# lukasc-ch/CBinfer

Hardware: AMD Instinct MI355X
Metric: frames/sec + effective GFLOP/s vs dense, scene-labeling CNN 480x320 @10% change (higher is better)
Workload: dtype f32-equivalent: f32 tensors, every operand as three bf16 terms (24 bits, exact), six products on the bf16 MFMA, f32 accumulate; 1 GPU; sceneLabeling CBConv2d coarse-grained fp32, synthetic 480x320 seq @10% change (32x32 re-drawn blocks), experiment 6, one sequence per GPU; sequences_per_gpu=1, launch=program

## Files before the change

cbinfer_amd/csrc/cb_split.hip:

```cpp
#include <stdlib.h>

#include <type_traits>

#include "cb_common.h"

#ifdef CBS_STAMP
__device__ unsigned long long cbs_stamp_buf[4 * 2048 * 16];
#define CB_TAIL_STAMP(i)                                                                 \
    do {                                                                                 \
        if (threadIdx.x == 0 && blockIdx.x < 2048)                                       \
            cbs_stamp_buf[(2 * 2048 + blockIdx.x) * 16 + (i)] = __builtin_amdgcn_s_memrealtime(); \
    } while (0)
#define CBS_DET_STAMP(i)                                                                                            \
    do {                                                                                                            \
        const unsigned wg = blockIdx.y * gridDim.x + blockIdx.x;                                                    \
        if (POOL && threadIdx.x == 0 && blockIdx.z == 0 && wg < 2048)                                               \
            cbs_stamp_buf[(3 * 2048 + wg) * 16 + (i)] = __builtin_amdgcn_s_memrealtime();                            \
    } while (0)
#else
#define CBS_DET_STAMP(i)
#endif
#include "cb_tail_core.h"
#include "cb_split_common.h"

namespace cbs {

typedef __attribute__((address_space(3))) void* cb_lds_ptr;

__global__ __launch_bounds__(256) void cbs_prep_kernel(const float* __restrict__ w, halfx8* __restrict__ A,
                                                      int* __restrict__ stageOff, float* __restrict__ wPlain,
                                                      CbsGeom g, int K, int KP, float wscale) {
    const long idx = (long)blockIdx.x * blockDim.x + threadIdx.x;
    if (wPlain)
        for (long i = idx; i < (long)K * g.C * g.kH * g.kW; i += (long)gridDim.x * blockDim.x) wPlain[i] = w[i];
    const int PL = g.planes;
    if (idx < g.nStages) {
        const int s = (int)idx;
        int off;
        if (g.pair) {
            off = ((s / g.kWs) * g.Wp + 2 * (s % g.kWs)) * g.rec;
// ... 240 lines not shown
struct CbsSeq {
    const char* S;
    const float* state;
    const int* rangeFlag;
    float* out;
    unsigned long long* masks;
    int32_t* listOut;
    int32_t* countOut;
    unsigned long long* maskCopy;
    float* reluOut;
};
struct CbsParams {
    CbsSeq seq[CBS_MAXSEQ];
    int nSeq;
    const char* A;
    const int* stageOff;
    const float* wPlain;
    const float* bias;
    float* slabs;
    int* info;
    int slabCap;
    int K, KP, H, W, Wp, rec, nStages, maskWords, wpr, relu, dummyBase, kH, kW;
    long stateBytes, aBytes;
    float outScale;
    unsigned long long magicMW, magicWpr, magicW, magicMT;
    int arriveShards;
    int forceSK;
    int accumulate;
    int splitRounds;
    int halfOut;
    const int* upstream;
    int dbg;
    int maxChunks;
};
static __device__ __forceinline__ const void* cbs_uniform_ptr(const void* ptr) {
    const unsigned long a = (unsigned long)ptr;
    const unsigned lo = (unsigned)__builtin_amdgcn_readfirstlane((int)(unsigned)a);
    const unsigned hi = (unsigned)__builtin_amdgcn_readfirstlane((int)(unsigned)(a >> 32));
    return (const void*)(((unsigned long)hi << 32) | lo);
}
#define CBH_GROUP CBINFER_HGROUP_MAX
#define CBH_NEXT CBINFER_HNEXT_MAX
struct CbhNext {
    _Float16* state;
    char* S;
    unsigned long long* masks;
    int kHH, kWH, Wp, rec, padY, padXL;
    float th;
    int pad_;
};
struct CbhLayer {
    const char* A;
    const _Float16* bias;
    int K, relu, nNext, pad_;
    CbhNext next[CBH_NEXT];
};
struct CbhExt {
    CbhLayer L[CBH_GROUP];
    int slabCap1;
    int pad_;
};
struct CbsNoExt {};
struct CbsWinExt {
    float* nstate;
    char* nS;
    unsigned long long* nmasks;
// ... 18 lines not shown
struct CbsExtOf<3> {
    typedef CbsWinExt type;
};
struct CbsSideExt {
    const float* sideFrame;
    float* sideState;
    int sideC, sideHW;
    float sideTh;
};
template <>
struct CbsExtOf<4> {
    typedef CbsSideExt type;
};

__device__ __forceinline__ void cbh_or_dilated(unsigned long long* masks, int y, int x, int H, int W, int wpr, int kHH,
                                               int kWH) {
    const int lo = max(x - kWH, 0), hi = min(x + kWH, W - 1);
    const int w0 = lo >> 6, w1 = hi >> 6;
    const unsigned long long m0 = (~0ull << (lo & 63)) & (w1 == w0 ? (~0ull >> (63 - (hi & 63))) : ~0ull);
    const unsigned long long m1 = ~0ull >> (63 - (hi & 63));
    for (int yy = max(y - kHH, 0); yy <= min(y + kHH, H - 1); ++yy) {
        atomicOr(&masks[(long)yy * wpr + w0], m0);
        if (w1 != w0) atomicOr(&masks[(long)yy * wpr + w1], m1);
    }
}

#ifdef CBS_STAMP
#define CBS_STAMP_AT(i)                                                                                   \
    do {                                                                                                  \
        if (threadIdx.x == 0 && blockIdx.x < 2048 && cbs_first)                                           \
            cbs_stamp_buf[(BM >= 128 ? 2048 * 16 : 0) + blockIdx.x * 16 + (i)] =                            \
                ((i) == 6 || (i) == 7) ? __builtin_amdgcn_s_memtime() : __builtin_amdgcn_s_memrealtime();               \
    } while (0)
#else
#define CBS_STAMP_AT(i)
#endif
#ifdef CBS_DBG
#define CBS_DBGBIT(b) (p.dbg & (b))
#else
#define CBS_DBGBIT(b) false
#endif
#define CBS_INFO_SK 0
#define CBS_INFO_MT 1
#define CBS_INFO_TP 4
#define CBS_INFO_CH 24

template <int OFF>
__device__ __forceinline__ void cbs_dma16(__amdgpu_buffer_rsrc_t rsrc, char* lds, int voff, int soff) {
    __builtin_amdgcn_raw_ptr_buffer_load_lds(rsrc, (cb_lds_ptr)lds, 16, voff, soff, OFF, 0);
}

template <int OFF>
__device__ __forceinline__ halfx8 cbs_lds_read16(unsigned addr) {
    halfx8 v;
    asm volatile("ds_read_b128 %0, %1 offset:%2" : "=v"(v) : "v"(addr), "n"(OFF));
    return v;
}

__device__ __forceinline__ int cbs_div(int x, unsigned long long magic) {
    return (int)(((unsigned long long)(unsigned)x * magic) >> 32);
}

template <int BM, int BN, int WM, int WN, int PRE_CAP, bool MASK_LDS, int RING, int AR = 0>
__global__ __launch_bounds__(64 * WM * WN) void cbs_conv_kernel(CbsParams p, typename CbsExtOf<AR>::type ext) {
    constexpr bool HALF = AR == 1, X3 = AR == 2 || AR == 3 || AR == 4, WIN = AR == 3, SIDE = AR == 3 || AR == 4;
    if (HALF && p.upstream && *p.upstream == 0) {
        if (blockIdx.x == 0 && threadIdx.x == 0) {
            p.seq[0].countOut[0] = 0;
            if (p.info) p.info[CBS_INFO_SK] = 1;
        }
        return;
    }
    cb_touch_kernarg<sizeof(CbsParams) + (HALF ? sizeof(CbhExt) : (WIN ? sizeof(CbsWinExt) : (SIDE ? sizeof(CbsSideExt) : 0)))>();
    constexpr int NW = WM * WN, NT = 64 * NW;
    constexpr int TN = BN / WN / 32;
    static_assert(BM == 32 * WM, "one 32-row tile per wave");
    constexpr int PB = X3 ? 192 : 128;
    constexpr int ABLK = BM * PB / 1024, BBLK = BN * PB / 1024;
    constexpr int APW = ABLK / NW, BPW = BBLK / NW;
    static_assert(APW * NW == ABLK && BPW * NW == BBLK && APW >= 1 && BPW >= 1, "DMA blocks must deal evenly");
    constexpr int DPW = APW + BPW;
    constexpr int A_BYTES = BM * PB, B_BYTES = BN * PB, STAGE = A_BYTES + B_BYTES;
    constexpr int TILE = BM * BN;
    __shared__ __attribute__((aligned(1024))) char ring[RING * STAGE];
    __shared__ int s_pre[PRE_CAP + 1];
    __shared__ unsigned long long s_mask[MASK_LDS ? PRE_CAP : 1];
    __shared__ const unsigned long long* s_maskPtr[CBS_MAXSEQ];
    __shared__ int s_wsum[NW];
    __shared__ int s_tilePix[BN];
    __shared__ float s_bias[BM];
    __shared__ unsigned s_nchg[HALF ? CBH_NEXT * (BN / 32) : 1];
    __shared__ int s_preW[WIN ? PRE_CAP / 2 + 2 : 1];
    __shared__ int s_tileAny[WIN ? BN : 1];
    __shared__ int s_winPos[WIN ? BN / 4 : 1];
    __shared__ unsigned s_wchg;
    __shared__ unsigned long long s_wsum64[WIN ? 64 * WM * WN / 64 : 1];
    static_assert(!WIN || (BN / WN / 32 == 1 && MASK_LDS), "window order: one column tile per wave, the mask words in LDS");

    const int t = threadIdx.x;
    const int lane = t & 63, wave = __builtin_amdgcn_readfirstlane(t >> 6);
    const int wm = wave % WM, wn = wave / WM;
    const int l31 = lane & 31, h = lane >> 5;
// ... 401 lines not shown
                    v += outx[(long)m * HWx + pix];
                    float* rp = pp->seq[q].reluOut;
                    if (rp) rp[(long)m * HWx + pix] = v <= 0.f ? 0.f : v;
                }
                outx[(long)m * HWx + pix] = v;
            }
            continue;
        }

        const char* Sq = p.seq[q].S;
        const int bRecords = (int)min(p.stateBytes + CBS_SPAD, (long)0x7fffffff);
        const int aVoff = wave * APW * 1024 + lane * 16;
        int bVoff[BPW];
#pragma unroll
        for (int i = 0; i < BPW; ++i) {
            const int nl = X3 ? wave * 16 + (lane >> 2) : (wave * BPW + i) * 8 + (lane >> 3);
            const int pos = s_tilePix[nl];
            const int py = cbs_div(max(pos, 0), p.magicW);
            const int base = (pos < 0 || CBS_DBGBIT(1)) ? p.dummyBase : (py * p.Wp + (pos - py * p.W)) * p.rec;
            if (X3)
                bVoff[i] = CBS_SPAD + base + ((i * 4 + ((lane & 3) ^ ((lane >> 4) & 3))) << 4) - i * 1024;
            else
                bVoff[i] = CBS_SPAD + base + (((lane & 7) ^ ((nl >> 1) & 7)) << 4) - (APW + i) * 1024;
        }
        const int aItem = (m0 / 32) * (PB * 32);
        const int aStageBytes = (p.KP / 32) * (PB * 32);

        CBS_STAMP_AT(11);
        __amdgpu_buffer_rsrc_t isA, isB;
        char* isMine = ring;
        int isAS = 0, isBS = 0;
        auto issue = [&](int s, bool setUpOnly = false) {
            char* dst = ring + (s % RING) * STAGE;
            const bool live = s < sEnd;
            const int aS = live ? s * aStageBytes + aItem : 0;
            const int bS = bNext;
            bNext = stageOff[min(s + 1, sEnd - 1)];
            if (CBS_DBGBIT(4)) return;
            const __amdgpu_buffer_rsrc_t ar = __builtin_amdgcn_make_buffer_rsrc(
                (void*)Aq, 0, (live && !CBS_DBGBIT(64 | 128)) ? aRecords : 0, 0x00020000);
            const __amdgpu_buffer_rsrc_t br = __builtin_amdgcn_make_buffer_rsrc(
                (void*)Sq, 0, (live && !CBS_DBGBIT(64 | 256)) ? bRecords : 0, 0x00020000);
            char* mine = dst + wave * (DPW * 1024);
            if (setUpOnly) {
                isA = ar, isB = br, isMine = mine, isAS = aS, isBS = bS;
                return;
            }
            if constexpr (X3) {
                cbs_dma16<0>(ar, mine, aVoff, aS);
                cbs_dma16<1024>(ar, mine, aVoff, aS);
                cbs_dma16<2048>(ar, mine, aVoff, aS);
                cbs_dma16<0>(br, mine + 3072, bVoff[0], bS);
                cbs_dma16<1024>(br, mine + 3072, bVoff[BPW > 1 ? 1 : 0], bS);
                cbs_dma16<2048>(br, mine + 3072, bVoff[BPW > 2 ? 2 : 0], bS);
            } else {
                cbs_dma16<0>(ar, mine, aVoff, aS);
                cbs_dma16<1024>(ar, mine, aVoff, aS);
                cbs_dma16<2048>(br, mine, bVoff[0], bS);
                cbs_dma16<3072>(br, mine, bVoff[1], bS);
            }
        };

        auto issuePart = [&](auto partTag) {
            constexpr int I = decltype(partTag)::value;
            if (CBS_DBGBIT(4)) return;
            if constexpr (X3) {
                if constexpr (I == 0) cbs_dma16<0>(isA, isMine, aVoff, isAS);
// ... 186 lines not shown
                asm volatile("s_waitcnt lgkmcnt(0)"
                             : "+v"(f.a[0]), "+v"(f.a[1]), "+v"(f.a[2]), "+v"(f.a[3]), "+v"(f.b[0]), "+v"(f.b[1]),
                               "+v"(f.b[2]), "+v"(f.b[3])
                             :
                             : "memory");
        };
#define CBS_SB() __builtin_amdgcn_sched_barrier(0)
#define CBS_STEP(WAITN, ISSUE, S, FCUR, FNEXT)                                            \
        do {                                                                               \
            asm volatile("s_waitcnt vmcnt(%0)" ::"n"(WAITN) : "memory");                  \
            __builtin_amdgcn_s_barrier();                                                  \
            CBS_SB();                                                                      \
            if (ISSUE) issue((S) + RING, true);                                            \
            CBS_SB();                                                                      \
            mmaRange(FCUR, 0, 1); CBS_SB(); if (ISSUE) issuePart(P0()); CBS_SB();          \
            mmaRange(FCUR, 1, 2); CBS_SB(); if (ISSUE) issuePart(P1()); CBS_SB();          \
            mmaRange(FCUR, 2, 3); CBS_SB();                                                \
            readA((S) + 1, FNEXT); CBS_SB(); if (ISSUE) issuePart(P2t()); CBS_SB();        \
            mmaRange(FCUR, 3, 4); CBS_SB();                                                \
            readB((S) + 1, FNEXT, 0); CBS_SB(); if (ISSUE) issuePart(P3()); CBS_SB();      \
            mmaRange(FCUR, 4, 5);                                                          \
            CBS_SB();                                                                      \
            if (TN > 1) readB((S) + 1, FNEXT, TN - 1);                                     \
            CBS_SB();                                                                      \
            mmaRange(FCUR, 5, NM);                                                         \
            waitFrags(FNEXT);                                                              \
        } while (0)

        typedef std::integral_constant<int, 0> KS0;
        typedef std::integral_constant<int, 1> KS1;
        typedef std::integral_constant<int, 6> R6;
        typedef std::integral_constant<int, 7> R7;
        typedef std::integral_constant<int, 8> R8;
#define CBS_STEP3A(S, FCUR, FNEXT)                                                         \
        do {                                                                               \
            CBS_SB();                                                                      \
            mma3(KS0(), FCUR, 0, 1); CBS_SB(); read1(KS1(), P0(), (S), FNEXT); read1(KS1(), P3(), (S), FNEXT); CBS_SB(); \
            mma3(KS0(), FCUR, 1, 2); CBS_SB(); read1(KS1(), P1(), (S), FNEXT); read1(KS1(), P4(), (S), FNEXT); CBS_SB(); \
            mma3(KS0(), FCUR, 2, 3); CBS_SB(); read1(KS1(), P2t(), (S), FNEXT); read1(KS1(), P5(), (S), FNEXT); CBS_SB(); \
            mma3(KS0(), FCUR, 3, 4); CBS_SB(); read1(KS1(), R6(), (S), FNEXT); CBS_SB();   \
            mma3(KS0(), FCUR, 4, 5); CBS_SB(); read1(KS1(), R7(), (S), FNEXT); CBS_SB();   \
            mma3(KS0(), FCUR, 5, 6); CBS_SB(); read1(KS1(), R8(), (S), FNEXT); CBS_SB();   \
            mma3(KS0(), FCUR, 6, NM3);                                                     \
            waitFrags(FNEXT);                                                              \
        } while (0)
#define CBS_STEP3B(WAITN, S, FCUR, FNEXT)                                                  \
        do {                                                                               \
            asm volatile("s_waitcnt vmcnt(%0)" ::"n"(WAITN) : "memory");                  \
            __builtin_amdgcn_s_barrier();                                                  \
            CBS_SB();                                                                      \
            issue((S) + RING, true);                                                       \
            CBS_SB();                                                                      \
            mma3(KS1(), FCUR, 0, 1); CBS_SB();                                             \
            read1(KS0(), P0(), (S) + 1, FNEXT); read1(KS0(), P3(), (S) + 1, FNEXT); CBS_SB(); issuePart(P0()); CBS_SB(); \
            mma3(KS1(), FCUR, 1, 2); CBS_SB();                                             \
            read1(KS0(), P1(), (S) + 1, FNEXT); read1(KS0(), P4(), (S) + 1, FNEXT); CBS_SB(); issuePart(P1()); CBS_SB(); \
            mma3(KS1(), FCUR, 2, 3); CBS_SB();                                             \
            read1(KS0(), P2t(), (S) + 1, FNEXT); read1(KS0(), P5(), (S) + 1, FNEXT); CBS_SB(); issuePart(P2t()); CBS_SB(); \
            mma3(KS1(), FCUR, 3, 4); CBS_SB(); read1(KS0(), R6(), (S) + 1, FNEXT); CBS_SB(); issuePart(P3()); CBS_SB(); \
            mma3(KS1(), FCUR, 4, 5); CBS_SB(); read1(KS0(), R7(), (S) + 1, FNEXT); CBS_SB(); issuePart(P4()); CBS_SB(); \
            mma3(KS1(), FCUR, 5, 6); CBS_SB(); read1(KS0(), R8(), (S) + 1, FNEXT); CBS_SB(); issuePart(P5()); CBS_SB(); \
            mma3(KS1(), FCUR, 6, NM3);                                                     \
            waitFrags(FNEXT);                                                              \
        } while (0)

        constexpr bool NEXT_REGS = HALF && TN == 1;
        _Float16 hv16[NEXT_REGS ? 16 : 1], sv16[NEXT_REGS ? CBH_NEXT : 1][NEXT_REGS ? 16 : 1];
        if constexpr (NEXT_REGS) {
            if (nNext > 0 && SK == 1) {
                const int pixLd = max(s_tilePix[wn * 32 + l31], 0);
                const int nx2 = nNext > 1 ? 1 : 0;
                const int mb0 = m0 + wm * 32 + 4 * h;
#pragma unroll
                for (int r = 0; r < 16; ++r) {
                    const long o = (long)min(mb0 + 8 * (r >> 2) + (r & 3), Kq - 1) * HW + pixLd;
                    sv16[0][r] = ext.L[q].next[0].state[o];
                    if (CBH_NEXT > 1) sv16[CBH_NEXT > 1 ? 1 : 0][r] = ext.L[q].next[nx2].state[o];
                }
            }
        }
        float oldv[WIN ? 16 : 1], nsv[WIN ? 4 : 1];
        int anyPos = -1, wPos = -1;
        if constexpr (WIN) {
            const int nl = wn * 32 + l31;
            anyPos = s_tileAny[nl], wPos = s_winPos[nl >> 2];
            const int aLd = max(anyPos, 0), wLd = max(wPos, 0);
            const long H2W2 = (long)ext.H2 * ext.W2;
            const float* oq = p.seq[0].out;
            if (__builtin_amdgcn_ballot_w64(anyPos >= 0 && s_tilePix[nl] < 0) != 0ull) {
#pragma unroll
                for (int r = 0; r < 16; ++r) {
                    const int m = min(wm * 32 + (r & 3) + 8 * (r >> 2) + 4 * h, Kq - 1);
                    oldv[r] = oq[(long)m * HW + aLd];
                }
            } else {
#pragma unroll
                for (int r = 0; r < 16; ++r) oldv[r] = 0.f;
            }
            const int c0 = wm * 32 + 8 * (nl & 3) + 4 * h;
#pragma unroll
            for (int e = 0; e < 4; ++e) nsv[e] = ext.nstate[(long)min(c0 + e, Kq - 1) * H2W2 + wLd];
        }
        Frags F0, F1;
        CBS_STAMP_AT(2);
#pragma unroll
        for (int i = 0; i < RING; ++i) issue(sBeg + i);
        asm volatile("s_waitcnt vmcnt(%0)" ::"n"((RING - 1) * DPW) : "memory");
        __builtin_amdgcn_s_barrier();
        __builtin_amdgcn_sched_barrier(0);
        if constexpr (X3) {
            readA3(KS0(), sBeg, F0);
#pragma unroll
            for (int j = 0; j < TN; ++j) readB3(KS0(), sBeg, F0, j);
        } else {
            readFrags(sBeg, F0);
        }
        waitFrags(F0);
        if (t < BM) s_bias[t] = biasv;
        CBS_STAMP_AT(3);
        int s = sBeg;
        if constexpr (X3) {
            for (int c = c0; c < c1; ++c) {
                const int cEnd = chunkBeg(c + 1);
                for (; s < cEnd; ++s) {
                    CBS_STEP3A(s, F0, F1);
                    CBS_STEP3B((RING - 2) * DPW, s, F1, F0);
                }
                if (c + 1 < c1) fold();
            }
        }
        if constexpr (!X3) {
            for (int c = c0; c < c1; ++c) {
                const int cEnd = chunkBeg(c + 1);
                for (; s + 1 < cEnd; s += 2) {
                    CBS_STEP((RING - 2) * DPW, true, s, F0, F1);
                    CBS_STEP((RING - 2) * DPW, true, s + 1, F1, F0);
                }
                if (c + 1 < c1) fold();
            }
            if (s < sEnd) CBS_STEP((RING - 2) * DPW, true, s, F0, F1);
        }
        asm volatile("s_waitcnt vmcnt(0)" ::: "memory");
#undef CBS_STEP
#undef CBS_STEP3A
#undef CBS_STEP3B
#undef CBS_SB
        __builtin_amdgcn_sched_barrier(0);
        CBS_STAMP_AT(4);
        CBS_STAMP_AT(7);

        float* out = p.seq[q].out;
        int accum;
        float* reluPlane;
        {
            const char* ka = (const char*)__builtin_amdgcn_kernarg_segment_ptr();
            asm volatile("" : "+s"(ka));
            const CbsParams* pp = (const CbsParams*)ka;
            accum = pp->accumulate;
            reluPlane = accum ? pp->seq[q].reluOut : nullptr;
        }
        if (CBS_DBGBIT(32)) continue;
        if (SK > 1) {
            float4* slab = (float4*)p.slabs + (long)it * (TILE / 4);
#pragma unroll
            for (int j = 0; j < TN; ++j) {
                const int nl = (wn * TN + j) * 32 + l31;
#pragma unroll
                for (int r4 = 0; r4 < 4; ++r4) {
                    const int mq = wm * 8 + 2 * r4 + h;
                    slab[mq * BN + nl] = make_float4(comb(j, 4 * r4), comb(j, 4 * r4 + 1), comb(j, 4 * r4 + 2),
                                                     comb(j, 4 * r4 + 3));
                }
            }
            CBS_STAMP_AT(5);
#ifdef CBS_STAMP
            cbs_first = false;
#endif
            continue;
// ... 159 lines not shown
                            }
                            if (dm) {
#pragma unroll
                                for (int e = 0; e < 4; ++e)
                                    if ((dm >> e) & 1u) nst[(long)(mb + e) * HW + pix] = h16[4 * r4 + e];
                                if (mb < cpad) {
                                    typedef _Float16 halfx4 __attribute__((ext_vector_type(4)));
                                    *(halfx4*)(rec + mb * 2) =
                                        halfx4{h16[4 * r4], h16[4 * r4 + 1], h16[4 * r4 + 2], h16[4 * r4 + 3]};
                                }
                            }
                        }
                        if (chg) atomicOr(&s_nchg[c * (BN / 32) + (nl >> 5)], 1u << (nl & 31));
                    }
                }
                __syncthreads();
#pragma unroll 1
                for (int c = 0; c < nNext; ++c) {
                    const CbhNext& nx = ext.L[q].next[c];
                    if (t < BN && ((s_nchg[c * (BN / 32) + (t >> 5)] >> (t & 31)) & 1u)) {
                        const int pix = s_tilePix[t];
                        const int py = cbs_div(pix, p.magicW), px = pix - py * p.W;
                        cbh_or_dilated(nx.masks, py, px, p.H, p.W, p.wpr, nx.kHH, nx.kWH);
                    }
                }
            }
        }
        CBS_STAMP_AT(5);
#ifdef CBS_STAMP
        cbs_first = false;
#endif
    }

    if constexpr (SIDE) {
        if (ext.sideFrame) {
            const int busy = min(items, (int)gridDim.x), nIdle = (int)gridDim.x - busy;
            const bool idleDo = nIdle >= 32;
            const int parts = idleDo ? nIdle : (int)gridDim.x, part = idleDo ? (int)blockIdx.x - busy : (int)blockIdx.x;
            if (part >= 0) {
                const int per = (ext.sideHW + parts - 1) / parts;
                const int i1 = min(ext.sideHW, (part + 1) * per);
                for (int i = part * per + t; i < i1; i += NT) {
                    bool chg = false;
                    for (int c = 0; c < ext.sideC; ++c)
                        chg |= cb_changed(ext.sideState[(long)c * ext.sideHW + i], ext.sideFrame[(long)c * ext.sideHW + i],
                                          ext.sideTh);
                    if (chg)
                        for (int c = 0; c < ext.sideC; ++c)
                            ext.sideState[(long)c * ext.sideHW + i] = ext.sideFrame[(long)c * ext.sideHW + i];
                }
            }
        }
    }

    if (totAll == 0) return;
    __syncthreads();
    if (t == 0) {
        int* ctl = (int*)(p.seq[0].masks + 2 * (long)MW);
        const int nSh = p.arriveShards;
        int last = 0;
        if (nSh <= 1) {
            last = __hip_atomic_fetch_add(ctl + 2, 1, __ATOMIC_RELAXED, __HIP_MEMORY_SCOPE_AGENT) == (int)gridDim.x - 1;
        } else {
            const int sh = blockIdx.x % nSh, expected = ((int)gridDim.x - sh + nSh - 1) / nSh;
            int* c = (int*)(p.seq[0].masks + (long)MW) + sh * 32;
            if (__hip_atomic_fetch_add(c, 1, __ATOMIC_RELAXED, __HIP_MEMORY_SCOPE_AGENT) == expected - 1) {
                __hip_atomic_store(c, 0, __ATOMIC_RELAXED, __HIP_MEMORY_SCOPE_AGENT);
                const int active = min(nSh, (int)gridDim.x);
                last = __hip_atomic_fetch_add(ctl + 2, 1, __ATOMIC_RELAXED, __HIP_MEMORY_SCOPE_AGENT) == active - 1;
            }
        }
        s_wsum[0] = last;
    }
    __syncthreads();
    if (s_wsum[0]) {
        for (int i = t; i < E; i += NT) {
            const int q = cbs_div(i, p.magicMW), w = i - q * MW;
            ((unsigned long long*)s_maskPtr[q])[w] = 0ull;
        }
        if (t == 0) {
            int* ctl = (int*)(p.seq[0].masks + 2 * (long)MW);
            __hip_atomic_store(ctl + 2, 0, __ATOMIC_RELAXED, __HIP_MEMORY_SCOPE_AGENT);
        }
    }
}

__global__ __launch_bounds__(256) void cbs_reduce_kernel(CbsParams p, int BM, int BN) {
    cb_touch_kernarg<sizeof(CbsParams) + 8>();
    const int SK = p.info[CBS_INFO_SK];
    if (SK <= 1) return;
    const int MT = p.info[CBS_INFO_MT], CMB = MT * SK, TILE4 = BM * BN / 4, HW = p.H * p.W;
    int tilesBefore[CBS_MAXSEQ + 1];
    tilesBefore[0] = 0;
#pragma unroll
    for (int q = 0; q < CBS_MAXSEQ; ++q) tilesBefore[q + 1] = tilesBefore[q] + p.info[CBS_INFO_TP + q];
    const int TP = tilesBefore[CBS_MAXSEQ];
    const float4* __restrict__ slabs = (const float4*)p.slabs;
    const long total = (long)TP * MT * TILE4;
    for (long g = (long)blockIdx.x * 256 + threadIdx.x; g < total; g += (long)gridDim.x * 256) {
        const int tile = (int)(g / TILE4), c = (int)(g - (long)tile * TILE4);
        const int ptg = tile / MT, mt = tile % MT;
        const int nl = c % BN, mq = c / BN;
        int q = 0;
#pragma unroll
        for (int u = 1; u < CBS_MAXSEQ; ++u)
            if (u < p.nSeq && ptg >= tilesBefore[u]) q = u;
        const int n = (ptg - tilesBefore[q]) * BN + nl;
        const int N = p.info[CBS_INFO_TP + CBS_MAXSEQ + q];
        const float4* sl = slabs + ((long)ptg * CMB + mt) * TILE4 + c;
        const int pix = n < N ? p.seq[q].listOut[n] : -1;
        float s0 = 0.f, s1 = 0.f, s2 = 0.f, s3 = 0.f;
        for (int j0 = 0; j0 < SK; j0 += 8) {
            float4 v[8];
#pragma unroll
            for (int j = 0; j < 8; ++j)
                if (j0 + j < SK) v[j] = sl[(long)(j0 + j) * MT * TILE4];
#pragma unroll
            for (int j = 0; j < 8; ++j)
                if (j0 + j < SK) s0 += v[j].x, s1 += v[j].y, s2 += v[j].z, s3 += v[j].w;
        }
        if ((unsigned)pix >= (unsigned)HW) continue;
        const int m = mt * BM + 4 * mq;
        const float sv[4] = {s0, s1, s2, s3};
        float* out = p.seq[q].out;
#pragma unroll
        for (int e = 0; e < 4; ++e) {
            if (m + e >= p.K) continue;
            const float bv = !p.bias ? 0.f : (p.halfOut ? (float)((const _Float16*)p.bias)[m + e] : p.bias[m + e]);
            float v = fmaf(sv[e], p.outScale, bv);
            if (p.relu) v = v <= 0.f ? 0.f : v;
            if (p.halfOut) {
                ((_Float16*)out)[(long)(m + e) * HW + pix] = (_Float16)v;
                continue;
            }
            if (p.accumulate) {
                v += out[(long)(m + e) * HW + pix];
                float* rp = p.seq[q].reluOut;
                if (rp) rp[(long)(m + e) * HW + pix] = v <= 0.f ? 0.f : v;
            }
            out[(long)(m + e) * HW + pix] = v;
        }
    }
}

template <int BM, int BN>
__global__ __launch_bounds__(256) void cbh_reduce_kernel(CbsParams p, CbhExt ext) {
    cb_touch_kernarg<sizeof(CbsParams) + sizeof(CbhExt)>();
    if (p.info[CBS_INFO_SK] <= 1) return;
    const int MT = p.info[CBS_INFO_MT], TILE4 = BM * BN / 4, HW = p.H * p.W;
    int tilesBefore[CBH_GROUP + 1], slabBase[CBH_GROUP], chQ[CBH_GROUP];
    tilesBefore[0] = 0;
    {
        int run = 0;
#pragma unroll
        for (int q = 0; q < CBH_GROUP; ++q) {
            const int tq = p.info[CBS_INFO_TP + q];
            chQ[q] = p.info[CBS_INFO_CH + q];
            tilesBefore[q + 1] = tilesBefore[q] + tq;
            slabBase[q] = run;
            run += tq * MT * chQ[q];
        }
    }
    constexpr int PXG = 16, GP = BN / PXG;
    const int groups = tilesBefore[CBH_GROUP] * GP;
    const int t = threadIdx.x, px = t & 15;
    __shared__ unsigned s_chg[CBH_NEXT];
    const float4* __restrict__ slabs = (const float4*)p.slabs;
    const int QT = MT * (BM / 4);
    const int NCC = (QT + 31) / 32;
    for (int unit = blockIdx.x; unit < groups * NCC; unit += gridDim.x) {
        const int g = unit / NCC, cc = unit - g * NCC;
        const int ptg = g / GP, gi = g - ptg * GP;
        int q = 0;
#pragma unroll
        for (int u = 1; u < CBH_GROUP; ++u)
            if (u < p.nSeq && ptg >= tilesBefore[u]) q = u;
        const int n0 = (ptg - tilesBefore[q]) * BN + gi * PXG;
        const int N = p.info[CBS_INFO_TP + CBS_MAXSEQ + q];
        if (n0 >= N) continue;
        static_assert(CBH_GROUP == 2, "two layers");
        const int SK = q ? chQ[1] : chQ[0], CMB = MT * SK;
// ... 105 lines not shown
                if (c < nNext && chg[c]) atomicOr(&s_chg[c], 1u << px);
            __syncthreads();
            for (int c = 0; c < nNext; ++c) {
                const CbhNext& nx = L.next[c];
                const int dy = (t >> 4) - nx.kHH, yy = py + dy;
                if (pix >= 0 && ((s_chg[c] >> px) & 1u) && dy <= nx.kHH && yy >= 0 && yy < p.H)
                    cbh_or_dilated(nx.masks, yy, pxx, p.H, p.W, p.wpr, 0, nx.kWH);
            }
        }
    }
}

struct CbsTailArgs {
    const float* w1p;
    const float* b1;
    const float* w2;
    const float* b2;
    float* out[CBS_MAXSEQ];
    int C1, C2, relu1, relu2;
};
template <int BM, int BN>
__global__ __launch_bounds__(64 * CB_TAIL_MAXW) void cbs_reduce_tail_kernel(CbsParams p, CbsTailArgs ta) {
    extern __shared__ float cbs_tail_sm[];
    cb_touch_kernarg<sizeof(CbsParams) + sizeof(CbsTailArgs)>();
    const int C0 = p.K, C0P = (C0 + 15) / 16 * 16, C1 = ta.C1, C2 = ta.C2, HW = p.H * p.W;
    const int t = threadIdx.x, NT = blockDim.x;
    CB_TAIL_STAMP(0);
    const int SK = p.info[CBS_INFO_SK], MT = p.info[CBS_INFO_MT], CMB = MT * SK, TILE4 = BM * BN / 4;
    int tilesBefore[CBS_MAXSEQ + 1];
    tilesBefore[0] = 0;
#pragma unroll
    for (int q = 0; q < CBS_MAXSEQ; ++q) tilesBefore[q + 1] = tilesBefore[q] + p.info[CBS_INFO_TP + q];
    const int GP = BN / CB_TAIL_PX, groups = tilesBefore[CBS_MAXSEQ] * GP;
    if ((int)blockIdx.x >= groups) return;
    CB_TAIL_STAMP(1);
    const CbTailLds L = cb_tail_lds(cbs_tail_sm, C0P, C1, C2, NT);
    __shared__ int s_pix[CB_TAIL_PX];
    for (int i = t; i < C2 * C1; i += NT) L.W2s[i] = ta.w2[i];
    for (int i = t; i < C2; i += NT) L.b2s[i] = ta.b2[i];
    const float4* __restrict__ slabs = (const float4*)p.slabs;
    const bool hasBias = p.bias != nullptr;
    const float* biasp = hasBias ? p.bias : ta.b1;
    const int px = t & 15, cstep = NT >> 4;
    for (int g = blockIdx.x; g < groups; g += gridDim.x) {
        const int ptg = g / GP, gi = g - ptg * GP;
        int q = 0;
#pragma unroll
        for (int u = 1; u < CBS_MAXSEQ; ++u)
            if (u < p.nSeq && ptg >= tilesBefore[u]) q = u;
        const int nl0 = gi * CB_TAIL_PX, n0 = (ptg - tilesBefore[q]) * BN + nl0;
        const int N = p.info[CBS_INFO_TP + CBS_MAXSEQ + q];
        if (n0 >= N) continue;
        float* outq = p.seq[q].out;
        float* relq = p.accumulate ? p.seq[q].reluOut : nullptr;
        int pixMine = -1;
        if (n0 + px < N) pixMine = p.seq[q].listOut[n0 + px];
        int tq = t >> 4;
        asm volatile("" : "+v"(tq));
        if ((unsigned)pixMine >= (unsigned)HW) pixMine = -1;
        const int pixLd = max(pixMine, 0);
        if (SK > 1) {
            const float4* sl0 = slabs + (long)ptg * CMB * TILE4 + nl0 + px;
            const int QN = C0P / 4, rounds = (QN + 4 * cstep - 1) / (4 * cstep);
            for (int rd = 0; rd < rounds; ++rd) {
                const int cq0 = tq + rd * 4 * cstep;
                float4 v[4][CBS_CHUNKS], bq[4];
// ... 35 lines not shown
                            } else if (pixMine >= 0 && m < p.K) {
                                outq[(long)m * HW + pixMine] = r;
                            }
                            L.Xs[m * CB_TAIL_PX + px] = (m < p.K && pixMine >= 0) ? r : 0.f;
                        }
                    }
                }
            }
        } else {
            __syncthreads();
            if (t < CB_TAIL_PX) s_pix[t] = pixMine;
            const float* gsrc = relq ? relq : outq;
            for (int c0 = tq; c0 < C0P; c0 += 16 * cstep) {
                float v[16];
#pragma unroll
                for (int u = 0; u < 16; ++u) v[u] = gsrc[(long)min(c0 + u * cstep, C0 - 1) * HW + pixLd];
#pragma unroll
                for (int u = 0; u < 16; ++u) {
                    const int c = c0 + u * cstep;
                    if (c < C0P) L.Xs[c * CB_TAIL_PX + px] = (pixMine >= 0 && c < C0) ? v[u] : 0.f;
                }
            }
        }
        asm volatile("" ::: "memory");
        CbTailPre P;
        cb_tail_preload(P, ta.w1p, ta.b1, C0P, C1);
        CB_TAIL_STAMP(3);
        cb_tail_tile(L, s_pix, P, ta.w1p, ta.out[q], C0P, C1, C2, HW, ta.relu1, ta.relu2);
        CB_TAIL_STAMP(7);
    }
}

template <int BM, int BN, int WM, int WN, int PRE_CAP, bool MASK_LDS, int RING, int AR = 0>
int cbs_launch_conv(const CbsParams& p, int perCU, const CbsTailArgs* tail, hipStream_t s,
                    const typename CbsExtOf<AR>::type& ext = typename CbsExtOf<AR>::type()) {
    if ((long)p.nSeq * p.maskWords > PRE_CAP) return CB_ERR_UNSUPPORTED;
    const bool second = p.slabs && (p.nStages >= 48 || p.forceSK > 0);
    if (tail && !second) return CB_ERR_UNSUPPORTED;
    dim3 grid((unsigned)(perCU * cb_num_cus())), block(64 * WM * WN);
    hipLaunchKernelGGL((cbs_conv_kernel<BM, BN, WM, WN, PRE_CAP, MASK_LDS, RING, AR>), grid, block, 0, s, p, ext);
    int st = cb_launch_status();
    if (st != CB_OK) return st;
    if constexpr (AR == 1) {
        if (second) {
            hipLaunchKernelGGL((cbh_reduce_kernel<BM, BN>), dim3(2 * cb_num_cus()), dim3(256), 0, s, p, ext);
            st = cb_launch_status();
        }
        return st;
    }
    if (tail) {
        const int waves = (tail->C1 + 15) / 16;
        hipLaunchKernelGGL((cbs_reduce_tail_kernel<BM, BN>), dim3(2 * cb_num_cus()), dim3(64 * waves),
                           cb_tail_lds_bytes(p.K, tail->C1, tail->C2), s, p, *tail);
        st = cb_launch_status();
    } else if (second) {
        hipLaunchKernelGGL(cbs_reduce_kernel, dim3(4 * cb_num_cus()), dim3(256), 0, s, p, BM, BN);
        st = cb_launch_status();
    }
    return st;
}

}
using namespace cbs;

#ifdef CBS_STAMP
extern "C" int cbinfer_debug_split_stamps(void* host, long bytes, int clear) {
    if (clear) {
        void* d = nullptr;
        if (hipGetSymbolAddress(&d, HIP_SYMBOL(cbs_stamp_buf)) != hipSuccess) return -1;
        return (int)hipMemset(d, 0, sizeof(unsigned long long) * 4 * 2048 * 16);
    }
    return (int)hipMemcpyFromSymbol(host, HIP_SYMBOL(cbs_stamp_buf), (size_t)bytes);
}
#endif

extern "C" {

int cbinfer_split_supported(int C, int K, int kH, int kW) { return cbs_supported(C, K, kH, kW) ? 1 : 0; }
int cbinfer_split_max_sequences(void) { return CBS_MAXSEQ; }
long cbinfer_split_max_mask_words(int K) { return cbs_bm(K) >= 128 ? CBS_PRE_BIG : CBS_PRE_MID; }

long cbinfer_split_state_bytes(int C, int H, int W, int kH, int kW) {
    const CbsGeom g = cbs_geom(C, H, W, kH, kW);
    return CBS_SPAD + (long)g.Hp * g.Wp * g.rec;
}
long cbinfer_split3_state_bytes(int C, int H, int W, int kH, int kW) {
    const CbsGeom g = cbs_geom(C, H, W, kH, kW, 3);
    return CBS_SPAD + (long)g.Hp * g.Wp * g.rec;
}

static long cbs_plain_offset(long aBytes, int nStages) { return (aBytes + (long)nStages * 4 + 15) / 16 * 16; }
long cbinfer_split_prepared_bytes(int C, int K, int kH, int kW) {
    const CbsGeom g = cbs_geom(C, 64, 64, kH, kW);
    return cbs_plain_offset((long)g.nStages * (cbs_kp(K) / 32) * 4096, g.nStages) + (long)K * C * kH * kW * 4;
}
long cbinfer_split3_prepared_bytes(int C, int K, int kH, int kW) {
    const CbsGeom g = cbs_geom(C, 64, 64, kH, kW, 3);
    return cbs_plain_offset((long)g.nStages * (cbs_kp(K) / 32) * 6144, g.nStages);
}

static long cbs_slab_capacity(int nSeq, int H, int W, int K) {
    const int bm = cbs_bm(K), bn = bm >= 128 ? 128 : 64;
    const long tiles = (long)nSeq * (((long)H * W + bn - 1) / bn) * (cbs_kp(K) / bm);
// ... 781 lines not shown
```

Measured before the change: 11390 frames/s.

## Stagger X3 prologue loads and peel tail stages without dead ring issues

For the X3 (three-term bf16) path, the prologue now issues only two stages before starting MMAs when the item is long enough. It then issues the remaining ring stages inside the first few steps, so compute starts earlier instead of waiting for the full ring fill. The tail is peeled: the last RING stages run without issuing further loads and use waitcnt values matched to the remaining in-flight count, with a final mma3 epilogue. This removes the out-of-range dummy issues at the end. In exchange the code grows considerably and the counted-wait bookkeeping becomes more fragile, and the live predicate is now always true for X3.

Result: faster. 11530 frames/s (median of 6 runs) (+1.2%).

```diff
diff --git a/cbinfer_amd/csrc/cb_split.hip b/cbinfer_amd/csrc/cb_split.hip
--- a/cbinfer_amd/csrc/cb_split.hip
+++ b/cbinfer_amd/csrc/cb_split.hip
@@ -899,7 +899,7 @@
         int isAS = 0, isBS = 0;
         auto issue = [&](int s, bool setUpOnly = false) {
             char* dst = ring + (s % RING) * STAGE;
-            const bool live = s < sEnd;
+            const bool live = X3 || s < sEnd;
             const int aS = live ? s * aStageBytes + aItem : 0;
             const int bS = bNext;
             bNext = stageOff[min(s + 1, sEnd - 1)];
@@ -1152,37 +1152,53 @@
         typedef std::integral_constant<int, 6> R6;
         typedef std::integral_constant<int, 7> R7;
         typedef std::integral_constant<int, 8> R8;
-#define CBS_STEP3A(S, FCUR, FNEXT)                                                         \
+#define CBS_STEP3A(ISSUE, ISTAGE, S, FCUR, FNEXT)                                          \
         do {                                                                               \
             CBS_SB();                                                                      \
-            mma3(KS0(), FCUR, 0, 1); CBS_SB(); read1(KS1(), P0(), (S), FNEXT); read1(KS1(), P3(), (S), FNEXT); CBS_SB(); \
-            mma3(KS0(), FCUR, 1, 2); CBS_SB(); read1(KS1(), P1(), (S), FNEXT); read1(KS1(), P4(), (S), FNEXT); CBS_SB(); \
-            mma3(KS0(), FCUR, 2, 3); CBS_SB(); read1(KS1(), P2t(), (S), FNEXT); read1(KS1(), P5(), (S), FNEXT); CBS_SB(); \
-            mma3(KS0(), FCUR, 3, 4); CBS_SB(); read1(KS1(), R6(), (S), FNEXT); CBS_SB();   \
-            mma3(KS0(), FCUR, 4, 5); CBS_SB(); read1(KS1(), R7(), (S), FNEXT); CBS_SB();   \
-            mma3(KS0(), FCUR, 5, 6); CBS_SB(); read1(KS1(), R8(), (S), FNEXT); CBS_SB();   \
+            if (ISSUE) issue((ISTAGE), true);                                              \
+            CBS_SB();                                                                      \
+            mma3(KS0(), FCUR, 0, 1); CBS_SB(); read1(KS1(), P0(), (S), FNEXT); read1(KS1(), P3(), (S), FNEXT); CBS_SB(); if (ISSUE) issuePart(P0()); CBS_SB(); \
+            mma3(KS0(), FCUR, 1, 2); CBS_SB(); read1(KS1(), P1(), (S), FNEXT); read1(KS1(), P4(), (S), FNEXT); CBS_SB(); if (ISSUE) issuePart(P1()); CBS_SB(); \
+            mma3(KS0(), FCUR, 2, 3); CBS_SB(); read1(KS1(), P2t(), (S), FNEXT); read1(KS1(), P5(), (S), FNEXT); CBS_SB(); if (ISSUE) issuePart(P2t()); CBS_SB(); \
+            mma3(KS0(), FCUR, 3, 4); CBS_SB(); read1(KS1(), R6(), (S), FNEXT); CBS_SB(); if (ISSUE) issuePart(P3()); CBS_SB(); \
+            mma3(KS0(), FCUR, 4, 5); CBS_SB(); read1(KS1(), R7(), (S), FNEXT); CBS_SB(); if (ISSUE) issuePart(P4()); CBS_SB(); \
+            mma3(KS0(), FCUR, 5, 6); CBS_SB(); read1(KS1(), R8(), (S), FNEXT); CBS_SB(); if (ISSUE) issuePart(P5()); CBS_SB(); \
             mma3(KS0(), FCUR, 6, NM3);                                                     \
             waitFrags(FNEXT);                                                              \
         } while (0)
-#define CBS_STEP3B(WAITN, S, FCUR, FNEXT)                                                  \
+#define CBS_STEP3B(WAITN, ISSUE, ISTAGE, S, FCUR, FNEXT)                                   \
         do {                                                                               \
             asm volatile("s_waitcnt vmcnt(%0)" ::"n"(WAITN) : "memory");                  \
             __builtin_amdgcn_s_barrier();                                                  \
             CBS_SB();                                                                      \
-            issue((S) + RING, true);                                                       \
+            if (ISSUE) issue((ISTAGE), true);                                              \
             CBS_SB();                                                                      \
             mma3(KS1(), FCUR, 0, 1); CBS_SB();                                             \
-            read1(KS0(), P0(), (S) + 1, FNEXT); read1(KS0(), P3(), (S) + 1, FNEXT); CBS_SB(); issuePart(P0()); CBS_SB(); \
+            read1(KS0(), P0(), (S) + 1, FNEXT); read1(KS0(), P3(), (S) + 1, FNEXT); CBS_SB(); if (ISSUE) issuePart(P0()); CBS_SB(); \
             mma3(KS1(), FCUR, 1, 2); CBS_SB();                                             \
-            read1(KS0(), P1(), (S) + 1, FNEXT); read1(KS0(), P4(), (S) + 1, FNEXT); CBS_SB(); issuePart(P1()); CBS_SB(); \
+            read1(KS0(), P1(), (S) + 1, FNEXT); read1(KS0(), P4(), (S) + 1, FNEXT); CBS_SB(); if (ISSUE) issuePart(P1()); CBS_SB(); \
             mma3(KS1(), FCUR, 2, 3); CBS_SB();                                             \
-            read1(KS0(), P2t(), (S) + 1, FNEXT); read1(KS0(), P5(), (S) + 1, FNEXT); CBS_SB(); issuePart(P2t()); CBS_SB(); \
-            mma3(KS1(), FCUR, 3, 4); CBS_SB(); read1(KS0(), R6(), (S) + 1, FNEXT); CBS_SB(); issuePart(P3()); CBS_SB(); \
-            mma3(KS1(), FCUR, 4, 5); CBS_SB(); read1(KS0(), R7(), (S) + 1, FNEXT); CBS_SB(); issuePart(P4()); CBS_SB(); \
-            mma3(KS1(), FCUR, 5, 6); CBS_SB(); read1(KS0(), R8(), (S) + 1, FNEXT); CBS_SB(); issuePart(P5()); CBS_SB(); \
+            read1(KS0(), P2t(), (S) + 1, FNEXT); read1(KS0(), P5(), (S) + 1, FNEXT); CBS_SB(); if (ISSUE) issuePart(P2t()); CBS_SB(); \
+            mma3(KS1(), FCUR, 3, 4); CBS_SB(); read1(KS0(), R6(), (S) + 1, FNEXT); CBS_SB(); if (ISSUE) issuePart(P3()); CBS_SB(); \
+            mma3(KS1(), FCUR, 4, 5); CBS_SB(); read1(KS0(), R7(), (S) + 1, FNEXT); CBS_SB(); if (ISSUE) issuePart(P4()); CBS_SB(); \
+            mma3(KS1(), FCUR, 5, 6); CBS_SB(); read1(KS0(), R8(), (S) + 1, FNEXT); CBS_SB(); if (ISSUE) issuePart(P5()); CBS_SB(); \
             mma3(KS1(), FCUR, 6, NM3);                                                     \
             waitFrags(FNEXT);                                                              \
         } while (0)
+#define CBS_HEAD3(J)                                                                       \
+        if constexpr (RING - 2 > (J)) {                                                    \
+            CBS_STEP3A(true, sBeg + 2 * (J) + 2, s, F0, F1);                               \
+            CBS_STEP3B(((J) + 1) * DPW, true, sBeg + 2 * (J) + 3, s, F1, F0);              \
+            ++s;                                                                           \
+        }
+#define CBS_TAIL3(REM)                                                                     \
+        if constexpr (RING >= (REM)) {                                                     \
+            if (rem >= (REM)) {                                                            \
+                CBS_STEP3A(false, 0, s, F0, F1);                                           \
+                CBS_STEP3B(((REM) - 2) * DPW, false, 0, s, F1, F0);                        \
+                ++s;                                                                       \
+            }                                                                              \
+        }
 
         constexpr bool NEXT_REGS = HALF && TN == 1;
         _Float16 hv16[NEXT_REGS ? 16 : 1], sv16[NEXT_REGS ? CBH_NEXT : 1][NEXT_REGS ? 16 : 1];
@@ -1222,10 +1238,34 @@
             for (int e = 0; e < 4; ++e) nsv[e] = ext.nstate[(long)min(c0 + e, Kq - 1) * H2W2 + wLd];
         }
         Frags F0, F1;
+        constexpr int CBS_MIN_STAGES = 4;
+        constexpr bool HEAD3 = X3 && RING >= 5;
+        const bool staggered = HEAD3 && sEnd - sBeg >= 2 * RING - 2;
         CBS_STAMP_AT(2);
-#pragma unroll
-        for (int i = 0; i < RING; ++i) issue(sBeg + i);
-        asm volatile("s_waitcnt vmcnt(%0)" ::"n"((RING - 1) * DPW) : "memory");
+        if constexpr (HEAD3) {
+            __builtin_amdgcn_s_waitcnt(0x0F70);
+            if (t < BM) s_bias[t] = biasv;
+        }
+        if constexpr (X3) {
+            static_assert(RING >= 3 && RING <= 5 && RING - 1 <= CBS_MIN_STAGES, "the short item's burst; CBS_TAIL3(5..2) below");
+            if (staggered) {
+                issue(sBeg);
+                issue(sBeg + 1);
+                asm volatile("s_waitcnt vmcnt(%0)" ::"n"(DPW) : "memory");
+            } else if (RING <= CBS_MIN_STAGES || sEnd - sBeg >= RING) {
+#pragma unroll
+                for (int i = 0; i < RING; ++i) issue(sBeg + i);
+                asm volatile("s_waitcnt vmcnt(%0)" ::"n"((RING - 1) * DPW) : "memory");
+            } else {
+#pragma unroll
+                for (int i = 0; i < RING - 1; ++i) issue(sBeg + i);
+                asm volatile("s_waitcnt vmcnt(%0)" ::"n"((RING - 2) * DPW) : "memory");
+            }
+        } else {
+#pragma unroll
+            for (int i = 0; i < RING; ++i) issue(sBeg + i);
+            asm volatile("s_waitcnt vmcnt(%0)" ::"n"((RING - 1) * DPW) : "memory");
+        }
         __builtin_amdgcn_s_barrier();
         __builtin_amdgcn_sched_barrier(0);
         if constexpr (X3) {
@@ -1236,18 +1276,37 @@
             readFrags(sBeg, F0);
         }
         waitFrags(F0);
-        if (t < BM) s_bias[t] = biasv;
+        if constexpr (!HEAD3)
+            if (t < BM) s_bias[t] = biasv;
         CBS_STAMP_AT(3);
         int s = sBeg;
         if constexpr (X3) {
+            const int sTail = max(sBeg, sEnd - RING);
+            if constexpr (HEAD3) {
+                if (staggered) {
+                    CBS_HEAD3(0)
+                    CBS_HEAD3(1)
+                    CBS_HEAD3(2)
+                }
+            }
             for (int c = c0; c < c1; ++c) {
-                const int cEnd = chunkBeg(c + 1);
+                const int cEnd = min(chunkBeg(c + 1), sTail);
                 for (; s < cEnd; ++s) {
-                    CBS_STEP3A(s, F0, F1);
-                    CBS_STEP3B((RING - 2) * DPW, s, F1, F0);
+                    CBS_STEP3A(false, 0, s, F0, F1);
+                    CBS_STEP3B((RING - 2) * DPW, true, s + RING, s, F1, F0);
                 }
                 if (c + 1 < c1) fold();
             }
+            CBS_STAMP_AT(15);
+            const int rem = sEnd - s;
+            CBS_TAIL3(5)
+            CBS_TAIL3(4)
+            CBS_TAIL3(3)
+            CBS_TAIL3(2)
+            CBS_STEP3A(false, 0, s, F0, F1);
+            CBS_SB();
+            mma3(KS1(), F1, 0, NM3);
+            ++s;
         }
         if constexpr (!X3) {
             for (int c = c0; c < c1; ++c) {
@@ -1264,6 +1323,8 @@
 #undef CBS_STEP
 #undef CBS_STEP3A
 #undef CBS_STEP3B
+#undef CBS_TAIL3
+#undef CBS_HEAD3
 #undef CBS_SB
         __builtin_amdgcn_sched_barrier(0);
         CBS_STAMP_AT(4);
```

## Defer change-mask clearing from conv kernel exit to the following reduce kernels

Applied to the files above, without the earlier changes.

When a second (reduce or tail) kernel follows, the conv kernel now returns early instead of running its end-of-kernel control and mask-clear sequence. The mask words are zeroed instead by the reduce, cbh_reduce and reduce-tail kernels, spread over their grid in reverse block order. The aim is to take the serialized last-block cleanup off the conv kernel's critical path. The early path for a zero upstream count also resets per-sequence tile counts so the reduce kernels see zero work. This adds stores to the reduce kernels and relies on the conv kernel's control-counter handling being safe to skip.

Result: no change. 11430 frames/s before, 11470 frames/s after, median of 6 (+0.4%).

```diff
diff --git a/cbinfer_amd/csrc/cb_split.hip b/cbinfer_amd/csrc/cb_split.hip
--- a/cbinfer_amd/csrc/cb_split.hip
+++ b/cbinfer_amd/csrc/cb_split.hip
@@ -5,7 +5,7 @@
 #include "cb_common.h"
 
 #ifdef CBS_STAMP
-__device__ unsigned long long cbs_stamp_buf[4 * 2048 * 16];
+__device__ unsigned long long cbs_stamp_buf[5 * 2048 * 16];
 #define CB_TAIL_STAMP(i)                                                                 \
     do {                                                                                 \
         if (threadIdx.x == 0 && blockIdx.x < 2048)                                       \
@@ -312,6 +312,7 @@
     const int* upstream;
     int dbg;
     int maxChunks;
+    int clearLater;
 };
 static __device__ __forceinline__ const void* cbs_uniform_ptr(const void* ptr) {
     const unsigned long a = (unsigned long)ptr;
@@ -396,8 +397,14 @@
             cbs_stamp_buf[(BM >= 128 ? 2048 * 16 : 0) + blockIdx.x * 16 + (i)] =                            \
                 ((i) == 6 || (i) == 7) ? __builtin_amdgcn_s_memtime() : __builtin_amdgcn_s_memrealtime();               \
     } while (0)
+#define CBS_EXIT_STAMP(i)                                                                                 \
+    do {                                                                                                  \
+        if (threadIdx.x == 0 && blockIdx.x < 2048)                                                        \
+            cbs_stamp_buf[(4 * 2048 + blockIdx.x) * 16 + (BM >= 128 ? 8 : 0) + (i)] = __builtin_amdgcn_s_memrealtime(); \
+    } while (0)
 #else
 #define CBS_STAMP_AT(i)
+#define CBS_EXIT_STAMP(i)
 #endif
 #ifdef CBS_DBG
 #define CBS_DBGBIT(b) (p.dbg & (b))
@@ -431,7 +438,10 @@
     if (HALF && p.upstream && *p.upstream == 0) {
         if (blockIdx.x == 0 && threadIdx.x == 0) {
             p.seq[0].countOut[0] = 0;
-            if (p.info) p.info[CBS_INFO_SK] = 1;
+            if (p.info) {
+                p.info[CBS_INFO_SK] = 1;
+                for (int q = 0; q < CBH_GROUP; ++q) p.info[CBS_INFO_TP + q] = 0;
+            }
         }
         return;
     }
@@ -1489,6 +1499,7 @@
 #endif
     }
 
+    CBS_EXIT_STAMP(0);
     if constexpr (SIDE) {
         if (ext.sideFrame) {
             const int busy = min(items, (int)gridDim.x), nIdle = (int)gridDim.x - busy;
@@ -1510,7 +1521,16 @@
         }
     }
 
+    CBS_EXIT_STAMP(1);
     if (totAll == 0) return;
+    {
+        const char* ka = (const char*)__builtin_amdgcn_kernarg_segment_ptr();
+        asm volatile("" : "+s"(ka));
+        if (((const CbsParams*)ka)->clearLater) {
+            CBS_EXIT_STAMP(2);
+            return;
+        }
+    }
     __syncthreads();
     if (t == 0) {
         int* ctl = (int*)(p.seq[0].masks + 2 * (long)MW);
@@ -1540,18 +1560,30 @@
             __hip_atomic_store(ctl + 2, 0, __ATOMIC_RELAXED, __HIP_MEMORY_SCOPE_AGENT);
         }
     }
+    CBS_EXIT_STAMP(2);
+}
+
+__device__ __forceinline__ void cbs_clear_masks(const CbsParams& p, int tilesAll) {
+    if (tilesAll == 0) return;
+    const int first = ((int)gridDim.x - 1 - (int)blockIdx.x) * (int)blockDim.x + (int)threadIdx.x;
+    if (first >= p.maskWords) return;
+    for (int q = 0; q < p.nSeq; ++q) {
+        unsigned long long* m = p.seq[q].masks;
+        for (int i = first; i < p.maskWords; i += (int)(gridDim.x * blockDim.x)) m[i] = 0ull;
+    }
 }
 
 __global__ __launch_bounds__(256) void cbs_reduce_kernel(CbsParams p, int BM, int BN) {
     cb_touch_kernarg<sizeof(CbsParams) + 8>();
     const int SK = p.info[CBS_INFO_SK];
+    int tilesBefore[CBS_MAXSEQ + 1];
+    tilesBefore[0] = 0;
+#pragma unroll
+    for (int q = 0; q < CBS_MAXSEQ; ++q) tilesBefore[q + 1] = tilesBefore[q] + p.info[CBS_INFO_TP + q];
+    const int TP = tilesBefore[CBS_MAXSEQ];
+    cbs_clear_masks(p, TP);
     if (SK <= 1) return;
     const int MT = p.info[CBS_INFO_MT], CMB = MT * SK, TILE4 = BM * BN / 4, HW = p.H * p.W;
-    int tilesBefore[CBS_MAXSEQ + 1];
-    tilesBefore[0] = 0;
-#pragma unroll
-    for (int q = 0; q < CBS_MAXSEQ; ++q) tilesBefore[q + 1] = tilesBefore[q] + p.info[CBS_INFO_TP + q];
-    const int TP = tilesBefore[CBS_MAXSEQ];
     const float4* __restrict__ slabs = (const float4*)p.slabs;
     const long total = (long)TP * MT * TILE4;
     for (long g = (long)blockIdx.x * 256 + threadIdx.x; g < total; g += (long)gridDim.x * 256) {
@@ -1603,7 +1635,14 @@
 template <int BM, int BN>
 __global__ __launch_bounds__(256) void cbh_reduce_kernel(CbsParams p, CbhExt ext) {
     cb_touch_kernarg<sizeof(CbsParams) + sizeof(CbhExt)>();
-    if (p.info[CBS_INFO_SK] <= 1) return;
+    const int SKany = p.info[CBS_INFO_SK];
+    {
+        int tilesAll = 0;
+#pragma unroll
+        for (int q = 0; q < CBH_GROUP; ++q) tilesAll += p.info[CBS_INFO_TP + q];
+        cbs_clear_masks(p, tilesAll);
+    }
+    if (SKany <= 1) return;
     const int MT = p.info[CBS_INFO_MT], TILE4 = BM * BN / 4, HW = p.H * p.W;
     int tilesBefore[CBH_GROUP + 1], slabBase[CBH_GROUP], chQ[CBH_GROUP];
     tilesBefore[0] = 0;
@@ -1775,6 +1814,7 @@
 #pragma unroll
     for (int q = 0; q < CBS_MAXSEQ; ++q) tilesBefore[q + 1] = tilesBefore[q] + p.info[CBS_INFO_TP + q];
     const int GP = BN / CB_TAIL_PX, groups = tilesBefore[CBS_MAXSEQ] * GP;
+    cbs_clear_masks(p, tilesBefore[CBS_MAXSEQ]);
     if ((int)blockIdx.x >= groups) return;
     CB_TAIL_STAMP(1);
     const CbTailLds L = cb_tail_lds(cbs_tail_sm, C0P, C1, C2, NT);
@@ -1876,12 +1916,13 @@
 }
 
 template <int BM, int BN, int WM, int WN, int PRE_CAP, bool MASK_LDS, int RING, int AR = 0>
-int cbs_launch_conv(const CbsParams& p, int perCU, const CbsTailArgs* tail, hipStream_t s,
+int cbs_launch_conv(CbsParams& p, int perCU, const CbsTailArgs* tail, hipStream_t s,
                     const typename CbsExtOf<AR>::type& ext = typename CbsExtOf<AR>::type()) {
     if ((long)p.nSeq * p.maskWords > PRE_CAP) return CB_ERR_UNSUPPORTED;
     const bool second = p.slabs && (p.nStages >= 48 || p.forceSK > 0);
     if (tail && !second) return CB_ERR_UNSUPPORTED;
     dim3 grid((unsigned)(perCU * cb_num_cus())), block(64 * WM * WN);
+    p.clearLater = second ? 1 : 0;
     hipLaunchKernelGGL((cbs_conv_kernel<BM, BN, WM, WN, PRE_CAP, MASK_LDS, RING, AR>), grid, block, 0, s, p, ext);
     int st = cb_launch_status();
     if (st != CB_OK) return st;
@@ -1912,7 +1953,7 @@
     if (clear) {
         void* d = nullptr;
         if (hipGetSymbolAddress(&d, HIP_SYMBOL(cbs_stamp_buf)) != hipSuccess) return -1;
-        return (int)hipMemset(d, 0, sizeof(unsigned long long) * 4 * 2048 * 16);
+        return (int)hipMemset(d, 0, sizeof(unsigned long long) * 5 * 2048 * 16);
     }
     return (int)hipMemcpyFromSymbol(host, HIP_SYMBOL(cbs_stamp_buf), (size_t)bytes);
 }
```
